# mitsuba-renderer/mitsuba2

Hardware: AMD Instinct MI355X
Metric: Msamples/sec (whole node), 1080p/512spp path integrator (higher is better)
Workload: dtype f32

## Files before the change

### mitsuba2_amd/csrc/device/film_kernels.h

```cpp
__global__ void k_film_resolve(const double *accum, float *out32, double *out64, size_t n, int accumulate) {
    size_t i = (size_t) blockIdx.x * blockDim.x + threadIdx.x;
    if (i >= n) return;
    if (out64) out64[i] = accumulate ? out64[i] + accum[i] : accum[i];
    else out32[i] = accumulate ? (float) ((double) out32[i] + accum[i]) : (float) accum[i];
}

#define MIW_FP_SIDE 8
#define MIW_FP_MAXN 8
struct PatchArgs { uint32_t patches_x, patches_y; int32_t reach; };

template <bool wide>
__global__ __launch_bounds__(64) void k_film_blocks(FilmRec F, BlockReplayArgs A, PatchArgs PA, float *tiles) {
    __shared__ float s_lut[MIW_FILTER_RESOLUTION + 1];
    __shared__ float s_w[64 * 2 * MIW_FP_MAXN];
    const uint32_t l = threadIdx.x;
    const uint32_t tile = blockIdx.x / (PA.patches_x * PA.patches_y), patch = blockIdx.x % (PA.patches_x * PA.patches_y);
    const uint32_t b = A.tile_list ? A.tile_list[tile] : tile;
    const BlockGeom g = block_geom(F, A.blocks_x, b);
    const int ptx0 = (int) (patch % PA.patches_x) * MIW_FP_SIDE, pty0 = (int) (patch / PA.patches_x) * MIW_FP_SIDE;
    if (ptx0 >= g.size_x || pty0 >= g.size_y) return;
    const int tx = ptx0 + (int) (l & 7u), ty = pty0 + (int) (l >> 3);
    if (l < 32) s_lut[l] = F.lut[l];
    __syncthreads();

// ... 563 lines not shown
#pragma unroll
            for (int p = P0; p <= P1; ++p) { wx[p].x = px[2 * p]; wx[p].y = px[2 * p + 1]; }
#pragma unroll
            for (int q = R0; q <= R1; ++q) {
                const float wy = py[q];
#pragma unroll
                for (int p = P0; p <= P1; ++p) {
                    const miw_f2 w = wy * wx[p];
                    film_pk_acc(acc[q][p][0], vx * w); film_pk_acc(acc[q][p][1], vy * w); film_pk_acc(acc[q][p][2], vz * w);
                    film_pk_acc(acc[q][p][3], af * w);
                    film_pk_acc(acc[q][p][4], w);
                }
#if MIW_FL_FENCE
                __builtin_amdgcn_sched_barrier(0);
#endif
            }
        }
    }
}
#ifndef MIW_FL_WAVES
#define MIW_FL_WAVES 3
#endif
template <int U, int NT, int WV = MIW_FL_WAVES>
__global__ __launch_bounds__(64) __attribute__((amdgpu_waves_per_eu(WV, 8))) void k_film_lanes(FilmRec F, BlockReplayArgs A, PatchArgs PA , uint32_t n_tiles, float *tiles,
                  uint32_t group0 ,
                  uint32_t prio ) {
    if (prio == 3u) __builtin_amdgcn_s_setprio(3); else if (prio == 2u) __builtin_amdgcn_s_setprio(2); else if (prio == 1u) __builtin_amdgcn_s_setprio(1);
    constexpr int BS = MIW_FL_BS, WS = MIW_FQ_WSTRIDE(MIW_FL_BS), LEAD = BS - 1, LCAP = 64;
    extern __shared__ float s_w[];
    __shared__ unsigned short s_list[LCAP];
    const uint32_t l = threadIdx.x;
    const uint32_t n_pos = PA.patches_x * PA.patches_y;
    const uint32_t tw = blockIdx.x / n_pos + group0, pos = blockIdx.x % n_pos;
    const int tx0 = (int) (pos % PA.patches_x) * BS, ty0 = (int) (pos / PA.patches_x) * BS;
    const uint32_t tile = tw * 64u + l;
    const bool live = tile < n_tiles;
    const BlockGeom g = block_geom(F, A.blocks_x, live ? (A.tile_list ? A.tile_list[tile] : tile) : 0u);
    const uint32_t rej = A.cls.count;
    const int reach = A.cls.reach;
    for (uint32_t i = l; i < (rej + 1u) * WS; i += 64u) {
        const uint32_t c = i / WS, a = i % WS;
        s_w[i] = (c < rej && a >= (uint32_t) LEAD && a <= (uint32_t) LEAD + 2u * (uint32_t) reach) ? A.cls.w[c * MIW_FC_STRIDE + a - LEAD] : 0.f;
    }
    const uint32_t bs2 = 1u << A.bs2_log2;
    uint32_t fill = 0;
    for (uint32_t q0 = 0; q0 < bs2; q0 += 64u) {
        const uint32_t q = q0 + l;
        uint32_t x, y;
        morton_decode2(q, x, y);
        const bool in = q < bs2 && (int) x >= tx0 - F.border - reach && (int) x <= tx0 + BS - 1 - F.border + reach &&
                        (int) y >= ty0 - F.border - reach && (int) y <= ty0 + BS - 1 - F.border + reach;
        const unsigned long long m = __ballot(in);
        if (in) {
            const uint32_t at = fill + (uint32_t) __popcll(m & ((1ull << l) - 1ull));
            if (at < (uint32_t) LCAP) s_list[at] = (unsigned short) q;
        }
        fill += (uint32_t) __popcll(m);
    }
    const uint32_t n_list = fill < (uint32_t) LCAP ? fill : (uint32_t) LCAP;
    __syncthreads();

    miw_f2 acc[BS][BS / 2][MIW_FILM_CHANNELS];
#pragma unroll
    for (int r = 0; r < BS; ++r)
#pragma unroll
        for (int p = 0; p < BS / 2; ++p)
#pragma unroll
            for (int k = 0; k < MIW_FILM_CHANNELS; ++k) acc[r][p][k] = (miw_f2) (0.f);
    const uint32_t w_base = (uint32_t) (uintptr_t) (miw_lds_cf *) s_w;
    const uint32_t off_rej = rej * (uint32_t) (WS * 4);
    const uint32_t lane0 = tile << A.bs2_log2;
    const uint32_t js = A.log_il ? 64u : 1u;
    struct Step { const U4 *run; uint32_t cnt; };
    auto pixel_at = [&](uint32_t k) { return (uint32_t) __builtin_amdgcn_readfirstlane((int) (k < n_list ? (uint32_t) s_list[k] : 0u)); };
    auto step_of = [&](uint32_t k, uint32_t q) {
        Step s; s.run = A.log_rec; s.cnt = 0u;
        uint32_t x, y;
        morton_decode2(q, x, y);
        if (k < n_list && live && (int) x < g.bw && (int) y < g.bh) { s.cnt = A.st[lane0 + q].w; s.run = A.log_rec + log_index(A.log_il, lane0 + q, A.spp, 0u); }
        return s;
    };
    uint4 nxt[U];
    auto fetch = [&](const U4 *run, uint32_t cnt) {
        const uint32_t last = cnt ? cnt - 1u : 0u;
#pragma unroll
        for (int i = 0; i < U; ++i) {
            nxt[i] = film_load_rec<NT>(run + ((uint32_t) i < last ? (uint32_t) i : last) * js);
            __builtin_amdgcn_sched_barrier(0);
        }
    };
    uint32_t q = pixel_at(0u);
    Step cur = step_of(0u, q);
    fetch(cur.run, cur.cnt);
    for (uint32_t k = 0; k < n_list; ++k) {
        const uint32_t step_max = (uint32_t) __builtin_amdgcn_readfirstlane((int) wave_max_u32(cur.cnt));
        const uint32_t qn = pixel_at(k + 1u);
        const Step nx = step_of(k + 1u, qn);
        uint32_t x, y;
        morton_decode2(q, x, y);
        const int ax = tx0 - ((int) x + F.border - reach), ay = ty0 - ((int) y + F.border - reach);
        const int c0 = ax < 0 ? -ax : 0, c1 = 2 * reach - ax < BS - 1 ? 2 * reach - ax : BS - 1;
        const int r0 = ay < 0 ? -ay : 0, r1 = 2 * reach - ay < BS - 1 ? 2 * reach - ay : BS - 1;
        const uint32_t bxa = w_base + 4u * (uint32_t) (LEAD + ax), bya = w_base + 4u * (uint32_t) (LEAD + ay);
        const int code = __builtin_amdgcn_readfirstlane(((r0 * 4 + r1) * 2 + (c0 >> 1)) * 2 + (c1 >> 1));
#define MIW_FL_CASE(R0, R1, P0, P1) case ((R0 * 4 + R1) * 2 + P0) * 2 + P1: \
            film_lanes_pixel<R0, R1, P0, P1, U, NT>(acc, nxt, cur.cnt, nx.run, nx.cnt, cur.run, step_max, bxa, bya, off_rej, js); break;
#define MIW_FL_ROWS(R0, R1) MIW_FL_CASE(R0, R1, 0, 0) MIW_FL_CASE(R0, R1, 0, 1) MIW_FL_CASE(R0, R1, 1, 1)
        switch (code) {
            MIW_FL_ROWS(0, 0) MIW_FL_ROWS(0, 1) MIW_FL_ROWS(0, 2) MIW_FL_ROWS(0, 3) MIW_FL_ROWS(1, 1) MIW_FL_ROWS(1, 2) MIW_FL_ROWS(1, 3)
            MIW_FL_ROWS(2, 2) MIW_FL_ROWS(2, 3) MIW_FL_ROWS(3, 3)
            default: break;
        }
#undef MIW_FL_ROWS
#undef MIW_FL_CASE
        if (step_max == 0u) fetch(nx.run, nx.cnt);
        cur = nx; q = qn;
    }
#pragma unroll
    for (int r = 0; r < BS; ++r)
#pragma unroll
        for (int c = 0; c < BS; ++c)
            if (live && tx0 + c < g.size_x && ty0 + r < g.size_y) {
                float *out = tiles + (size_t) tile * A.tile_stride + ((size_t) (ty0 + r) * g.size_x + (tx0 + c)) * MIW_FILM_CHANNELS;
#pragma unroll
                for (int k = 0; k < MIW_FILM_CHANNELS; ++k) out[k] = (c & 1) ? acc[r][c / 2][k].y : acc[r][c / 2][k].x;
            }
}

__global__ void k_film_merge(FilmRec F, BlockReplayArgs A, const float *tiles, float *out32, double *out64, int accumulate) {
    int fx = (int) (blockIdx.x * blockDim.x + threadIdx.x), fy = (int) blockIdx.y;
    if (fx >= F.crop_w || fy >= F.crop_h) return;
    float v[MIW_FILM_CHANNELS];
    size_t o = ((size_t) fy * F.crop_w + fx) * MIW_FILM_CHANNELS;
    if (accumulate) for (int k = 0; k < MIW_FILM_CHANNELS; ++k) v[k] = out64 ? (float) out64[o + k] : out32[o + k];
    film_merge_texel(F, A, tiles, fx, fy, v, accumulate != 0);
    for (int k = 0; k < MIW_FILM_CHANNELS; ++k) {
        if (out64) out64[o + k] = (double) v[k]; else out32[o + k] = v[k];
    }
}
```

### mitsuba2_amd/csrc/miwave.hip

```cpp
#include <hip/hip_runtime.h>
#include <stdio.h>
#include <stdlib.h>
#include <string.h>
#include <stdarg.h>
#include <string>
#include <vector>
#include <chrono>
#include <atomic>
#include <cmath>
#include <map>
#include <string>
#include <algorithm>

#include "../../include/miwave.h"
#if defined(MIW_SECTION_PROFILE)
__device__ unsigned long long g_sections[16];
#endif
#if defined(MIW_PHASE_STATS)
__device__ unsigned long long g_phase_stats[15];
#endif
#if defined(MIW_WALK_STATS)
__device__ unsigned long long g_walk_stats[8];
__device__ float g_walk_statsf[8];
#endif
// ... 4 lines not shown
#if defined(MIW_SECTION_PROFILE) && defined(__HIP_DEVICE_COMPILE__)
__device__ __forceinline__ unsigned long long *miw_sec_buf() { __shared__ unsigned long long b[4][16]; return &b[threadIdx.x >> 6][0]; }
#define MIW_SECTION(i) do { const unsigned long long now_ = __builtin_amdgcn_s_memtime(); unsigned long long *b_ = miw_sec_buf(); \
        if ((threadIdx.x & 63u) == (unsigned) __ffsll((long long) __ballot(1)) - 1u) { b_[i] += now_ - b_[15]; b_[15] = now_; } } while (0)
#endif
#include "miw/base.h"
#include "miw/rng.h"
#include "miw/warp.h"
#include "miw/special.h"
#include "miw/shape.h"
#include "miw/bsdf.h"
#include "miw/scene.h"
#include "miw/film.h"
#include "miw/bvh.h"
#include "miw/path.h"
#include "miw/direct.h"
#include "rect_build.h"
#include "miw/film_gather.h"
#include "texture_build.h"
#include "bvh_build.h"
#include "bvh4_build.h"
#include "envmap_build.h"
#include "film_classes.h"
#include "lbvh_device.h"
#include "sah_device.h"
#include "bvh4_device.h"
#include "bvh8_device.h"
#include "film_reduce.h"

using namespace miw;

static_assert(sizeof(BvhNode) == 64, "BvhNode must be one 64-byte line");
static_assert(sizeof(Tri) == 48, "Tri must be 48 bytes");
static_assert(sizeof(BsdfRec) == 128 && sizeof(mi_bsdf) == 128, "bsdf record layout");
static_assert(sizeof(TexRec) == sizeof(mi_texture), "texture record layout");

#define MIW_BLOCK 256
#ifndef MIW_POOL_NW
#define MIW_POOL_NW 12
#endif
#define MIW_CNT_SHARDS 1024
#define MIW_BRUTE_MAX_LEAF 2
#define MIW_BRUTE_MAX_TRIS 64
#define MIW_PLACE_PIECES 4

#include "device/trace.h"
// ... 49 lines not shown
    { "MIW_PHASED", "0: tree scenes take the lock-step kernel instead of the phase machine" },
    { "MIW_PHASED_WAVES", "3 | 4: wavefronts per SIMD the phase machine is launched for" },
    { "MIW_TRIO", "0: MATS_PLAIN kernels where the MATS_TRIO class would do" },
    { "MIW_SHADE_VOTE", "num:den of the phase machine's shade vote" },
    { "MIW_LOOP_EXIT", "node:triangle hand-over ratios of the phase machine's walk loops" },
    { "MIW_POOLED", "1: tree scenes take k_path_pooled (walk jobs pooled across the workgroup; experimental, slower: DESIGN.md)" },
    { "MIW_POOL_SHAPE", "12x1 | 8x2: wavefronts per workgroup x pixels per lane of k_path_pooled" },
    { "MIW_POOL_VOTE", "shade_min:walk_min:node_min:tri_min:claim_min of k_path_pooled" },
    { "MIW_TAIL_PRIO", "0: no least-progress-first wave priorities" },
    { "MIW_WG_PER_CU", "workgroups per CU of the packet kernels' persistent grid" },
    { "MIW_PLACE", "0: shards of about one pixel per lane skip the measuring launch + placed queues" },
    { "MIW_JOB_CHUNK", "smallest chunk of a full frame's pixel jobs, in samples (a power of two; default 64, the phase machine 32): the pixels' sample streams are cut into halving chunks drawn chunk-major from one queue; 0: a job = all the samples of a pixel" },
    { "MIW_JOB_CHUNK_FORCE", "1: chunk jobs whatever the frame's size (tests of the hand-over between lanes)" },
    { "MIW_PACKET_SHARD4", "0: a plain-diffuse packet job of at most four wavefronts of pixels per SIMD keeps the five-wavefront (96-register) kernel" },
    { "MIW_PLACE_MEASURE", "divisor: the measuring launch runs spp / divisor samples" },
    { "MIW_PLACE_SPREAD", "0 | 1: placed pieces = consecutive sorted lanes | one lane of every cost stratum" },
    { "MIW_STREAM", "0: plan 1 walks with one kernel per list slice instead of the persistent stream kernel" },
    { "MIW_FILM_LEGACY", "1: the 24-byte position log + k_film_blocks for every filter" },
    { "MIW_FILM_LANES", "0 | 1 | 2: k_film_lanes off / over the tile-interleaved log / over [lane][sample]" },
    { "MIW_FILM_QUADS", "0 | 24 | 28 | 42 | 44: k_film_quads group shape (0: off)" },
    { "MIW_FILM_COLUMNS", "0 | 42 | 44 | 82: k_film_columns group shape" },
    { "MIW_FILM_GROUP", "2 | 3 | 4: k_film_groups group shape" },
    { "MIW_FL_NT", "0: k_film_lanes reads the log with plain instead of streaming loads" },
    { "MIW_FILM_OVERLAP", "1: part of the film replay of a full Cornell-class frame is queued on three more streams beside the path kernel, sets of 64-tile groups each behind the flags their last pixels raise (default 0: measured +0 - 1 %); 2: without the waits (timing probe: the film is the previous frame's)" },
    { "MIW_FILM_OVERLAP_SET", "groups of 64 tiles per launch of that replay (default 4)" },
    { "MIW_FILM_OVERLAP_ROOM", "workgroups the path kernel's grid is short of filling the device while the replay runs beside it (default 32: one per CU on 32 CUs)" },
    { "MIW_FILM_OVERLAP_LEAN", "0: the launches of that replay are the 168-register kernel (default 1: the 128-register form)" },
    { "MIW_FILM_OVERLAP_BESIDE", "groups of 64 tiles replayed beside the path kernel; the rest in one launch after it (default: three quarters)" },
    { "MIW_FILM_OVERLAP_PRIO", "s_setprio of the replay wavefronts that run beside the path kernel, 0 .. 3 (default 0)" },
    { "MIW_FQ_U", "2 | 4 | 8: records per trip of k_film_quads" },
    { "MIW_RCCL", "0: mi_film_reduce never uses RCCL (device add)" },
    { "MIW_RCCL_FORCE", "1: mi_film_reduce takes the RCCL branch for one context too (tests)" }
};
struct Options {
    std::map<std::string, std::string> v;
    void from_env() { for (const KnobInfo &k : g_knobs) if (const char *e = getenv(k.name)) v[k.name] = e; }
    static bool known(const char *name) { for (const KnobInfo &k : g_knobs) if (!strcmp(k.name, name)) return true; return false; }
    const char *get(const char *name) const { auto it = v.find(name); return it == v.end() ? nullptr : it->second.c_str(); }
};

struct mi_ctx {
    int device = 0;
    Options opt;
    hipStream_t stream = nullptr;
    std::string error;
    std::atomic<int> cancel{0};
// ... 19 lines not shown
    DevBuf<float> d_env_data, d_env_levels; DevBuf<EnvmapRec> d_env; EnvmapRec env_host{}; size_t env_levels_total = 0;
    bool have_env = false;
    SceneView view{};
    TraceLds lds_cfg{}; size_t lds_bytes = 0;

    DevBuf<F4> q_tp, q_res, q_ray_o, q_ray_d, q_hit, q_sh_d, q_sh_c;
    DevBuf<U4> q_st; DevBuf<F2> q_pos; DevBuf<uint32_t> q_pixel, q_sh_vis;
    DevBuf<double> d_accum; DevBuf<unsigned char> d_out;
    DevBuf<F2> q_log_pos; DevBuf<F4> q_log_val;
    DevBuf<U4> q_log_rec;
    FilmClasses classes; FilmRec classes_of{}; bool classes_valid = false;
    DevBuf<float> d_fc_thr, d_fc_w;
    DevBuf<uint32_t> d_next_pixel; int cu_count = 256;
    DevBuf<uint32_t> d_lane_cost, d_cost_sorted, d_lane_iota, d_lane_sorted, d_piece_list, d_simd_ids;
    DevBuf<unsigned char> d_place_tmp;
    DevBuf<uint32_t> d_lists, d_list_counts;
    DevBuf<uint32_t> d_block_ids, d_tile_list; DevBuf<int32_t> d_block_tile; DevBuf<float> d_tiles;
    DevBuf<Counters> d_cnt;
    Counters *h_cnt = nullptr;
    std::vector<uint32_t> h_piece_list, h_simd_ids;
    hipStream_t stream2[3] = { nullptr, nullptr, nullptr }; hipEvent_t ev_fork = nullptr, ev_join[3] = { nullptr, nullptr, nullptr };
    DevBuf<uint32_t> d_group_done, d_group_expected; uint32_t *h_group_flag = nullptr; uint32_t group_flag_cap = 0;
    std::vector<uint32_t> h_group_expected; std::vector<int32_t> h_block_tile;
    int overlap_state = -1;
    bool replay_enqueued = false;
    uint32_t replay_launches = 0;

    std::vector<hipEvent_t> ev_pool;
    mi_counters counters{};
};

static mi_status fail(mi_ctx *c, mi_status code, const char *fmt, ...) {
    char buf[512];
    va_list ap; va_start(ap, fmt); vsnprintf(buf, sizeof buf, fmt, ap); va_end(ap);
    if (c) c->error = buf;
    return code;
}
#define HIP_TRY(c, expr) do { hipError_t e_ = (expr); if (e_ != hipSuccess) \
    return fail(c, MI_ERR_DEVICE, "%s failed: %s (%s:%d)", #expr, hipGetErrorString(e_), __FILE__, __LINE__); } while (0)

static thread_local std::string g_global_error;

extern "C" {

int32_t mi_spectrum_channels(void) { return MIW_SPEC_N; }

// ... 12 lines not shown
    int n = 0;
    if (hipGetDeviceCount(&n) != hipSuccess || n <= 0) { g_global_error = "no HIP device visible"; return MI_ERR_DEVICE; }
    if (device < 0 || device >= n) { g_global_error = "device index out of range"; return MI_ERR_INVALID; }
    if (hipSetDevice(device) != hipSuccess) { g_global_error = "hipSetDevice failed"; return MI_ERR_DEVICE; }
    mi_ctx *c = new mi_ctx();
    c->device = device;
    c->opt.from_env();
    { hipDeviceProp_t prop; if (hipGetDeviceProperties(&prop, device) == hipSuccess && prop.multiProcessorCount > 0) c->cu_count = prop.multiProcessorCount; }
    if (hipHostMalloc((void **) &c->h_cnt, sizeof(Counters) * MIW_CNT_SHARDS) != hipSuccess) { delete c; g_global_error = "hipHostMalloc failed"; return MI_ERR_DEVICE; }
    *out = c;
    g_live_contexts.fetch_add(1);
    return MI_OK;
}

void mi_destroy(mi_ctx *c) {
    if (!c) return;
    (void) hipSetDevice(c->device);
    (void) hipDeviceSynchronize();
    c->d_nodes.release(); c->d_tris.release(); c->d_tri_vn.release(); c->d_tri_uv.release(); c->d_bitmap_data.release(); c->d_bitmaps.release(); c->d_bsdf_tables.release(); c->d_shapes.release(); c->d_rects.release(); c->d_bsdfs.release();
    c->d_emitters.release(); c->d_leaf_boxes.release(); c->d_tri_bounds.release(); c->d_nodes4.release(); c->d_nodes8.release(); c->d_tris8.release(); c->d_tri_vn8.release(); c->d_env_data.release(); c->d_env_levels.release(); c->d_env.release(); c->d_emit_tri.release(); c->d_emit_vnorm.release(); c->d_emit_pmf.release(); c->d_emit_cdf.release();
    c->q_tp.release(); c->q_res.release(); c->q_ray_o.release(); c->q_ray_d.release(); c->q_hit.release();
    c->q_sh_d.release(); c->q_sh_c.release(); c->q_st.release(); c->q_pos.release(); c->q_pixel.release(); c->q_sh_vis.release();
    c->d_accum.release(); c->d_out.release(); c->d_next_pixel.release(); c->d_lane_cost.release(); c->d_cost_sorted.release(); c->d_lane_iota.release(); c->d_lane_sorted.release(); c->d_place_tmp.release(); c->d_piece_list.release(); c->d_simd_ids.release(); c->d_lists.release(); c->d_list_counts.release(); c->d_block_ids.release(); c->d_tile_list.release(); c->d_cnt.release();
    c->q_log_pos.release(); c->q_log_val.release(); c->q_log_rec.release(); c->d_fc_thr.release(); c->d_fc_w.release(); c->d_block_tile.release(); c->d_tiles.release();
    for (hipEvent_t e : c->ev_pool) (void) hipEventDestroy(e);
    c->d_group_done.release(); c->d_group_expected.release();
    if (c->h_group_flag) (void) hipHostFree(c->h_group_flag);
    if (c->ev_fork) (void) hipEventDestroy(c->ev_fork);
    for (int i = 0; i < 3; ++i) { if (c->ev_join[i]) (void) hipEventDestroy(c->ev_join[i]); if (c->stream2[i]) (void) hipStreamDestroy(c->stream2[i]); }
    if (c->h_cnt) (void) hipHostFree(c->h_cnt);
    delete c;
    if (g_live_contexts.fetch_sub(1) == 1) rccl_release_comms();
}

mi_status mi_set_stream(mi_ctx *c, void *s) { if (!c) return MI_ERR_INVALID; c->stream = (hipStream_t) s; return MI_OK; }

const char *mi_last_error(mi_ctx *c) { return c ? c->error.c_str() : g_global_error.c_str(); }

mi_status mi_set_option(mi_ctx *c, const char *name, const char *value) {
    if (!c || !name) return MI_ERR_INVALID;
    if (!Options::known(name)) return fail(c, MI_ERR_INVALID, "mi_set_option: unknown option %s", name);
    if (value) c->opt.v[name] = value; else c->opt.v.erase(name);
    return MI_OK;
}
const char *mi_get_option(mi_ctx *c, const char *name) { return c && name ? c->opt.get(name) : nullptr; }
int32_t mi_option_count(void) { return (int32_t) (sizeof(g_knobs) / sizeof(g_knobs[0])); }
const char *mi_option_name(int32_t i) { return i >= 0 && i < mi_option_count() ? g_knobs[i].name : nullptr; }
// ... 964 lines not shown
                }
                memset(st, 0, sizeof st); memset(stf, 0, sizeof stf);
                (void) hipMemcpyToSymbol(HIP_SYMBOL(g_walk_stats), st, sizeof st); (void) hipMemcpyToSymbol(HIP_SYMBOL(g_walk_statsf), stf, sizeof stf);
            }
        }
#endif
#if defined(MIW_SECTION_PROFILE)
        if (ropt.get("MIW_DEBUG")) {
            unsigned long long sec[16];
            if (hipMemcpyFromSymbol(sec, HIP_SYMBOL(g_sections), sizeof sec) == hipSuccess) {
                static const char *names[13] = { "fetch/begin", "leaf boxes", "E candidates", "S candidates", "path_step", "finish+begin",
                                                 "walks + votes", "shade: surface interaction", "shade: emitter hit + MIS", "shade: RR + emitter sampling + bsdf eval",
                                                 "shade: bsdf sample", "shade: finish + next sample", "shade: pixel fetch + walk start" };
                unsigned long long tot = 0;
                for (int i = 0; i < 13; ++i) tot += sec[i];
                for (int i = 0; i < 13; ++i) if (sec[i]) fprintf(stderr, "[miwave] section %-40s %6.2f %%\n", names[i], 100.0 * (double) sec[i] / (double) std::max<unsigned long long>(tot, 1));
                memset(sec, 0, sizeof sec);
                (void) hipMemcpyToSymbol(HIP_SYMBOL(g_sections), sec, sizeof sec);
            }
        }
#endif
}

struct FilmReplay { BlockReplayArgs A; uint32_t side = 0; uint32_t beside = 0;  };
static mi_status film_replay_setup(mi_ctx *c, const mi_render_cfg *cfg, hipStream_t s, const FilmPlan &FP, uint32_t n_tiles, uint32_t bs, uint32_t bs2_log2,
                                   uint32_t blocks_x, uint32_t blocks_y, FilmReplay &R) {
    const bool rec16 = FP.rec16;
    std::vector<int32_t> &block_tile = c->h_block_tile;
    block_tile.assign(cfg->block_count, -1);
    for (uint32_t t = 0; t < n_tiles; ++t) block_tile[cfg->tile_list ? cfg->tile_list[t] : t] = (int32_t) t;
    HIP_TRY(c, c->d_block_tile.resize(cfg->block_count));
    HIP_TRY(c, hipMemcpyAsync(c->d_block_tile.p, block_tile.data(), block_tile.size() * sizeof(int32_t), hipMemcpyHostToDevice, s));
    BlockReplayArgs &A = R.A;
    A.log_pos = c->q_log_pos.p; A.log_val = c->q_log_val.p; A.st = c->q_st.p; A.spp = cfg->spp;
    A.log_rec = rec16 ? c->q_log_rec.p : nullptr; A.log_il = rec16 ? FP.log_il : 0u;
    A.cls.thr = c->d_fc_thr.p; A.cls.w = c->d_fc_w.p; A.cls.count = rec16 ? c->classes.count : 0u; A.cls.reach = rec16 ? c->classes.reach : 0;
    A.block_ids = c->d_block_ids.p; A.block_tile = c->d_block_tile.p;
    A.tile_list = cfg->tile_list ? c->d_tile_list.p : nullptr;
    A.blocks_x = blocks_x; A.blocks_y = blocks_y; A.bs2_log2 = bs2_log2;
    R.side = bs + 2u * (uint32_t) cfg->filter_border;
    A.tile_stride = R.side * R.side * MIW_FILM_CHANNELS;
    HIP_TRY(c, c->d_tiles.resize((size_t) std::max<uint32_t>(n_tiles, 1) * A.tile_stride));
    return MI_OK;
}

__global__ void k_raise_flags(uint32_t *flag, uint32_t n) {
    const uint32_t i = blockIdx.x * blockDim.x + threadIdx.x;
    if (i < n) __hip_atomic_store(flag + i, 1u, __ATOMIC_RELEASE, __HIP_MEMORY_SCOPE_SYSTEM);
}
static mi_status overlap_prepare(mi_ctx *c, const mi_render_cfg *cfg, hipStream_t s, uint32_t n_tiles, uint32_t bs, uint32_t blocks_x, LaneQueues &Q, uint32_t bs2_log2) {
    const uint32_t n_groups = (n_tiles + 63u) / 64u;
    if (!c->ev_fork) {
        bool ok = hipEventCreateWithFlags(&c->ev_fork, hipEventDisableTiming) == hipSuccess;
        for (int i = 0; i < 3 && ok; ++i)
            ok = hipStreamCreateWithFlags(&c->stream2[i], hipStreamNonBlocking) == hipSuccess && hipEventCreateWithFlags(&c->ev_join[i], hipEventDisableTiming) == hipSuccess;
        if (!ok) { (void) hipGetLastError(); c->overlap_state = 0; return MI_OK; }
    }
    if (c->group_flag_cap < n_groups) {
        if (c->h_group_flag) (void) hipHostFree(c->h_group_flag);
        c->h_group_flag = nullptr; c->group_flag_cap = 0;
        const uint32_t cap = std::max<uint32_t>(1024u, n_groups);
        if (hipHostMalloc((void **) &c->h_group_flag, cap * sizeof(uint32_t), hipHostMallocCoherent | hipHostMallocMapped) != hipSuccess) { (void) hipGetLastError(); c->overlap_state = 0; return MI_OK; }
        c->group_flag_cap = cap;
    }
    std::vector<uint32_t> &expected = c->h_group_expected;
    expected.assign(n_groups, 0u);
    for (uint32_t t = 0; t < n_tiles; ++t) {
        const uint32_t b = cfg->tile_list ? cfg->tile_list[t] : t, bx = b % blocks_x, by = b / blocks_x;
        const int32_t bw = std::min<int32_t>((int32_t) bs, cfg->crop_w - (int32_t) (bx * bs)), bh = std::min<int32_t>((int32_t) bs, cfg->crop_h - (int32_t) (by * bs));
        expected[t >> 6] += (uint32_t) (std::max(bw, 0) * std::max(bh, 0));
    }
    HIP_TRY(c, c->d_group_done.resize(n_groups)); HIP_TRY(c, c->d_group_expected.resize(n_groups));
    memset(c->h_group_flag, 0, n_groups * sizeof(uint32_t));
    HIP_TRY(c, hipMemsetAsync(c->d_group_done.p, 0, n_groups * sizeof(uint32_t), s));
    HIP_TRY(c, hipMemcpyAsync(c->d_group_expected.p, expected.data(), n_groups * sizeof(uint32_t), hipMemcpyHostToDevice, s));
    Q.group_done = c->d_group_done.p; Q.group_expected = c->d_group_expected.p; Q.group_flag = c->h_group_flag; Q.group_shift = bs2_log2 + 6u;
    return MI_OK;
}
static mi_status overlap_enqueue(mi_ctx *c, const Options &ropt, const RenderParams &P, hipStream_t s, LaunchTimer &T, FilmReplay &R, uint32_t n_tiles, bool wait_flags) {
    const uint32_t n_all = (n_tiles + 63u) / 64u;
    uint32_t n_groups = n_all * 3u / 4u;
    if (const char *e = ropt.get("MIW_FILM_OVERLAP_BESIDE")) n_groups = (uint32_t) std::min<long>(std::max<long>(atol(e), 0), (long) n_all);
    int prio = 0;
    if (const char *e = ropt.get("MIW_FILM_OVERLAP_PRIO")) prio = std::min(3, std::max(0, atoi(e)));
    PatchArgs PC; PC.patches_x = PC.patches_y = (R.side + MIW_FL_BS - 1) / MIW_FL_BS; PC.reach = c->classes.reach;
    const uint32_t n_pos = PC.patches_x * PC.patches_y;
    const size_t lbytes = (size_t) (c->classes.count + 1u) * MIW_FQ_WSTRIDE(MIW_FL_BS) * sizeof(float);
    int fl_nt = 1;
    if (const char *e = ropt.get("MIW_FL_NT")) fl_nt = atoi(e);
    uint32_t set = 4u;
    if (const char *e = ropt.get("MIW_FILM_OVERLAP_SET")) set = (uint32_t) std::max(1, atoi(e));
    bool lean_ok = fl_nt != 0;
    if (const char *e = ropt.get("MIW_FILM_OVERLAP_LEAN")) lean_ok = lean_ok && atoi(e) != 0;
    for (int i = 0; i < 3; ++i) HIP_TRY(c, hipStreamWaitEvent(c->stream2[i], c->ev_fork, 0));
    uint32_t launches = 0;
    for (uint32_t g0 = 0; g0 < n_groups; g0 += set, ++launches) {
        hipStream_t b = c->stream2[launches % 3u];
        const uint32_t g1 = std::min(n_groups, g0 + set);
        if (wait_flags)
            for (uint32_t g = g0; g < g1; ++g) {
                const hipError_t e = hipStreamWaitValue32(b, c->h_group_flag + g, 1u, hipStreamWaitValueGte, 0xffffffffu);
                if (e != hipSuccess) {
                    (void) hipGetLastError();
                    c->overlap_state = 0;
                    if (g == 0) return MI_OK;
                    return fail(c, MI_ERR_DEVICE, "hipStreamWaitValue32 failed mid-frame: %s", hipGetErrorString(e));
                }
            }
        size_t e0 = 0, e1 = 0;
        if (T.on) { HIP_TRY(c, T.get_event(e0)); HIP_TRY(c, hipEventRecord(c->ev_pool[e0], b)); }
        const bool lean = lean_ok;
        if (lean) hipLaunchKernelGGL((k_film_lanes<2, 1, 4>), dim3((g1 - g0) * n_pos), dim3(64), lbytes, b, P.film, R.A, PC, (uint32_t) n_tiles, c->d_tiles.p, g0, (uint32_t) prio);
        else if (fl_nt) hipLaunchKernelGGL((k_film_lanes<4, 1>), dim3((g1 - g0) * n_pos), dim3(64), lbytes, b, P.film, R.A, PC, (uint32_t) n_tiles, c->d_tiles.p, g0, (uint32_t) prio);
        else hipLaunchKernelGGL((k_film_lanes<4, 0>), dim3((g1 - g0) * n_pos), dim3(64), lbytes, b, P.film, R.A, PC, (uint32_t) n_tiles, c->d_tiles.p, g0, (uint32_t) prio);
        if (T.on) { HIP_TRY(c, T.get_event(e1)); HIP_TRY(c, hipEventRecord(c->ev_pool[e1], b)); T.stamps.push_back({ 4, e0, e1 }); }
    }
    for (int i = 0; i < 3; ++i) HIP_TRY(c, hipEventRecord(c->ev_join[i], c->stream2[i]));
    c->replay_launches = launches;
    R.beside = n_groups;
    hipLaunchKernelGGL(k_raise_flags, dim3((n_all + 255u) / 256u), dim3(256), 0, s, c->h_group_flag, n_all);
    HIP_TRY(c, hipGetLastError());
    c->replay_enqueued = true;
    c->overlap_state = 1;
    return MI_OK;
}

static mi_status assemble_film(mi_ctx *c, const mi_render_cfg *cfg, const Options &ropt, const RenderParams &P, hipStream_t s, LaunchTimer &T, const FilmPlan &FP,
                               uint32_t n_tiles, uint32_t bs, uint32_t bs2_log2, uint32_t blocks_x, uint32_t blocks_y, size_t film_n, void *film, mi_status result,
                               const FilmReplay *queued ) {
    const int film_mode = FP.film_mode; const bool rec16 = FP.rec16; const int film_lanes = FP.film_lanes; const uint32_t log_il = FP.log_il;
    (void) result;
#define MIW_TIMED(cls_, launch) do {                                                   \
        size_t e0_ = 0, e1_ = 0;                                                       \
        if (T.on) { HIP_TRY(c, T.get_event(e0_)); HIP_TRY(c, hipEventRecord(c->ev_pool[e0_], s)); } \
        launch;                                                                        \
        if (T.on) { HIP_TRY(c, T.get_event(e1_)); HIP_TRY(c, hipEventRecord(c->ev_pool[e1_], s)); \
                    T.stamps.push_back({ cls_, e0_, e1_ }); }                          \
    } while (0)
    {
        const size_t elem = cfg->film_f64 ? sizeof(double) : sizeof(float);
        void *dst = film;
        const bool staged = !cfg->film_on_device;
        if (staged) {
            HIP_TRY(c, c->d_out.resize(film_n * elem)); dst = c->d_out.p;
            if (cfg->accumulate) HIP_TRY(c, hipMemcpyAsync(c->d_out.p, film, film_n * elem, hipMemcpyHostToDevice, s));
        }
        float *dst32 = cfg->film_f64 ? nullptr : (float *) dst;
        double *dst64 = cfg->film_f64 ? (double *) dst : nullptr;
        if (film_mode == 1) {
            FilmReplay R;
            if (queued) R = *queued;
            else { const mi_status rs = film_replay_setup(c, cfg, s, FP, n_tiles, bs, bs2_log2, blocks_x, blocks_y, R); if (rs != MI_OK) return rs; }
            BlockReplayArgs &A = R.A;
            const uint32_t side = R.side;
            if (n_tiles) {
                PatchArgs PA;
                PA.patches_x = PA.patches_y = (side + MIW_FP_SIDE - 1) / MIW_FP_SIDE;
                PA.reach = (int32_t) floorf(cfg->filter_radius + .5f);
                const dim3 fgrid(n_tiles * PA.patches_x * PA.patches_y);
                const bool wide = cfg->filter_radius > 0.5f + MIW_RAY_EPSILON;
                if (rec16) {
                    int group = 3;
                    if (const char *e = ropt.get("MIW_FILM_GROUP")) group = atoi(e);
                    const size_t wbytes = (size_t) (c->classes.count + 1u) * MIW_FG_WSTRIDE * sizeof(float);
#define MIW_FG_LAUNCH(GW, GH) MIW_TIMED(4, hipLaunchKernelGGL((k_film_groups<GW, GH>), fgrid, dim3(64), wbytes, s, P.film, A, PA, c->d_tiles.p))
#define MIW_FC_LAUNCH(GW, GH) do { PatchArgs PC = PA; PC.patches_x = (side + (GW) - 1) / (GW); PC.patches_y = (side + (GH) - 1) / (GH); \
                                   const uint32_t per_wave = 64u / (GW), wpt = (PC.patches_x * PC.patches_y + per_wave - 1u) / per_wave; \
                                   MIW_TIMED(4, hipLaunchKernelGGL((k_film_columns<GW, GH>), dim3(n_tiles * wpt), dim3(64), wbytes, s, P.film, A, PC, c->d_tiles.p)); } while (0)
                    int columns = 42;
                    if (const char *e = ropt.get("MIW_FILM_COLUMNS")) columns = atoi(e);
                    int quads = ropt.get("MIW_FILM_COLUMNS") == nullptr && ropt.get("MIW_FILM_GROUP") == nullptr ? 42 : 0;
                    if (const char *e = ropt.get("MIW_FILM_QUADS")) quads = atoi(e) == 1 ? 42 : atoi(e);
                    if ((quads != 24 && quads != 42 && quads != 28 && quads != 44) || c->classes.reach > 2) quads = 0;
                    const uint32_t qw = (uint32_t) quads / 10u, qh = (uint32_t) quads % 10u;
                    if (quads && ((side + qw - 1) / qw) * ((side + qh - 1) / qh) < 64u / qw) quads = 0;
                    const bool lanes = film_lanes != 0;
                    c->counters.film_kernel = lanes ? 4u : quads ? 3u : (columns == 42 || columns == 44 || columns == 82) ? 2u : 1u;
                    if (lanes) {
                        PatchArgs PC = PA; PC.patches_x = PC.patches_y = (side + MIW_FL_BS - 1) / MIW_FL_BS;
                        const size_t lbytes = (size_t) (c->classes.count + 1u) * MIW_FQ_WSTRIDE(MIW_FL_BS) * sizeof(float);
                        int fl_nt = 1;
                        if (const char *e = ropt.get("MIW_FL_NT")) fl_nt = atoi(e);
                        const uint32_t first = queued ? queued->beside : 0u, groups_all = ((uint32_t) n_tiles + 63u) / 64u;
                        const uint32_t waves_rest = (groups_all - first) * PC.patches_x * PC.patches_y;
                        if (waves_rest == 0u) { }
                        else if (fl_nt) MIW_TIMED(4, hipLaunchKernelGGL((k_film_lanes<4, 1>), dim3(waves_rest), dim3(64), lbytes, s, P.film, A, PC, (uint32_t) n_tiles, c->d_tiles.p, first, 0u));
                        else MIW_TIMED(4, hipLaunchKernelGGL((k_film_lanes<4, 0>), dim3(waves_rest), dim3(64), lbytes, s, P.film, A, PC, (uint32_t) n_tiles, c->d_tiles.p, first, 0u));
                        if (queued) { for (int i = 0; i < 3; ++i) HIP_TRY(c, hipStreamWaitEvent(s, c->ev_join[i], 0)); }
                    } else if (quads) {
                        PatchArgs PC = PA; PC.patches_x = (side + qw - 1) / qw; PC.patches_y = (side + qh - 1) / qh;
                        const uint32_t per_wave = 64u / qw, waves = (uint32_t) (((size_t) n_tiles * PC.patches_x * PC.patches_y + per_wave - 1u) / per_wave);
                        const size_t qbytes = (size_t) (c->classes.count + 1u) * (size_t) (5u + 2u * qh) * sizeof(float);
#define MIW_FQ_LAUNCH(GW, GH, U) MIW_TIMED(4, hipLaunchKernelGGL((k_film_quads<GW, GH, U>), dim3(waves), dim3(64), qbytes, s, P.film, A, PC, (uint32_t) n_tiles, c->d_tiles.p))
                        int fq_u = 4;
                        if (const char *e = ropt.get("MIW_FQ_U")) fq_u = atoi(e);
                        if (quads == 24) { if (fq_u == 8) MIW_FQ_LAUNCH(2, 4, 8); else if (fq_u == 2) MIW_FQ_LAUNCH(2, 4, 2); else MIW_FQ_LAUNCH(2, 4, 4); }
                        else if (quads == 42) { if (fq_u == 8) MIW_FQ_LAUNCH(4, 2, 8); else MIW_FQ_LAUNCH(4, 2, 4); }
                        else if (quads == 28) MIW_FQ_LAUNCH(2, 8, 4); else MIW_FQ_LAUNCH(4, 4, 4);
#undef MIW_FQ_LAUNCH
                    } else if (columns == 42) MIW_FC_LAUNCH(4, 2); else if (columns == 44) MIW_FC_LAUNCH(4, 4); else if (columns == 82) MIW_FC_LAUNCH(8, 2);
                    else if (group == 4) MIW_FG_LAUNCH(4, 4); else if (group == 2) MIW_FG_LAUNCH(2, 2); else MIW_FG_LAUNCH(4, 2);
#undef MIW_FC_LAUNCH
#undef MIW_FG_LAUNCH
                } else if (wide)
                    MIW_TIMED(4, hipLaunchKernelGGL(k_film_blocks<true>, fgrid, dim3(64), 0, s, P.film, A, PA, c->d_tiles.p));
                else
                    MIW_TIMED(4, hipLaunchKernelGGL(k_film_blocks<false>, fgrid, dim3(64), 0, s, P.film, A, PA, c->d_tiles.p));
            }
            MIW_TIMED(5, hipLaunchKernelGGL(k_film_merge, dim3(((uint32_t) cfg->crop_w + 255u) / 256u, (uint32_t) cfg->crop_h), dim3(256), 0, s,
                                            P.film, A, c->d_tiles.p, dst32, dst64, cfg->accumulate));
// ... 246 lines not shown
            TA.side = 16u + 2u * std::max<uint32_t>((uint32_t) cfg->filter_border, (uint32_t) floorf(cfg->filter_radius + .5f));
            TA.geom16 = (uint32_t) ((c->lds_bytes + 15) / 16);
            tile_bytes = (size_t) TA.geom16 * 16 - c->lds_bytes + (size_t) TA.side * TA.side * MIW_FILM_CHANNELS * sizeof(double);
            if (c->lds_bytes + tile_bytes > 64 * 1024) {
                HIP_TRY(c, hipFuncSetAttribute((const void *) k_path_resident<false, 1>, hipFuncAttributeMaxDynamicSharedMemorySize, (int) (c->lds_bytes + tile_bytes)));
                HIP_TRY(c, hipFuncSetAttribute((const void *) k_path_resident<false, 0>, hipFuncAttributeMaxDynamicSharedMemorySize, (int) (c->lds_bytes + tile_bytes)));
                HIP_TRY(c, hipFuncSetAttribute((const void *) k_path_resident<false, 1, MATS_ALL, false, INTEG_DIRECT>, hipFuncAttributeMaxDynamicSharedMemorySize, (int) (c->lds_bytes + tile_bytes)));
                HIP_TRY(c, hipFuncSetAttribute((const void *) k_path_resident<false, 0, MATS_ALL, true, INTEG_DIRECT>, hipFuncAttributeMaxDynamicSharedMemorySize, (int) (c->lds_bytes + tile_bytes)));
            }
        }
        const uint32_t sync_every = 8;
        uint32_t launches = 0;
        bool place_stats_due = false;
        int overlap_mode = 0;
        if (const char *e = ropt.get("MIW_FILM_OVERLAP")) overlap_mode = atoi(e);
        const bool overlap = overlap_mode != 0 && c->overlap_state != 0 && film_mode == 1 && FP.rec16 && FP.film_lanes != 0 && FP.log_il != 0 && !place && !phased  && tiny && c->diffuse_only && !MIW_SPECTRAL && !direct  &&
                             per_launch >= cfg->spp && cfg->timeout_s <= 0.f && n_tiles > 0;
        for (uint32_t done = 0; done < cfg->spp; ) {
            uint32_t end = cfg->spp - done < per_launch ? cfg->spp : done + per_launch;
            if (film_mode == 1) {
                HIP_TRY(c, hipMemsetAsync(c->d_next_pixel.p, 0, c->d_next_pixel.n * sizeof(uint32_t), s));
                rcfg.queues = 1u; Q.lane_cost = nullptr; Q.lane_sorted = nullptr; Q.piece_list = nullptr; Q.simd_ids = nullptr;
                if (overlap && done == 0) {
                    mi_status os = film_replay_setup(c, cfg, s, FP, n_tiles, bs, bs2_log2, blocks_x, blocks_y, replay);
                    if (os == MI_OK) os = overlap_prepare(c, cfg, s, n_tiles, bs, blocks_x, Q, bs2_log2);
                    if (os != MI_OK) return os;
                    if (Q.group_done) HIP_TRY(c, hipEventRecord(c->ev_fork, s));
                }
                Q.job_chunk = Q.job_pow = Q.job_total = 0u; Q.job_min = 0x80000000u;
                if ((tiny || (phased && MIW_PHASED_JOBS != 0)) && !pooled_fits && !place && !overlap && done == 0 && per_launch >= cfg->spp && cfg->timeout_s <= 0.f) {
                    uint32_t jmin = tiny ? 64u : 32u;
                    if (const char *e = ropt.get("MIW_JOB_CHUNK")) { const uint32_t v = (uint32_t) std::max(0, atoi(e)); jmin = (v & (v - 1u)) ? 0u : v; }
                    bool enough = (uint64_t) n_lanes * 5u >= (uint64_t) 6u * 64u * res_waves * n_simd;
                    if (const char *e = ropt.get("MIW_JOB_CHUNK_FORCE")) enough = enough || atoi(e) != 0;
                    uint32_t pow2 = 1u;
                    while (pow2 * 2u < cfg->spp) pow2 *= 2u;
                    uint64_t chunks = 1u;
                    for (uint32_t r = pow2; jmin && r >= jmin && r < cfg->spp; r >>= 1) ++chunks;
                    if (jmin && enough && chunks >= 2u && (uint64_t) n_lanes * chunks < (1ull << 31)) {
                        Q.job_chunk = jmin; Q.job_min = jmin; Q.job_pow = pow2; Q.job_total = (uint32_t) ((uint64_t) n_lanes * chunks);
                        K.job_chunk = jmin; K.job_chunks = (uint32_t) chunks;
                    }
                }
                if (place && done == 0) { end = measure_end; Q.lane_cost = c->d_lane_cost.p; Q.simd_ids = c->d_simd_ids.p; }
                else if (place) {
                    HIP_TRY(c, rocprim::radix_sort_pairs_desc(c->d_place_tmp.p, place_tmp_bytes, c->d_lane_cost.p, c->d_cost_sorted.p, c->d_lane_iota.p, c->d_lane_sorted.p, (size_t) n_lanes, 0u, 32u, s));
                    bool spread = phased && ((phased8 ? (size_t) c->nodes8_count * sizeof(Bvh8Node) : (size_t) c->nodes4_count * sizeof(Bvh4Node)) + (size_t) c->view.tri_count * sizeof(Tri)) > ((size_t) 32 << 20);
// ... 304 lines not shown
```

Measured before the change: 4467.

## Pack film-lane block positions into equal-length chains per wavefront

The film replay kernel now processes a chain of up to four block positions per wavefront instead of one. A host-side bin packer groups positions so each chain has roughly equal pixel work, flushing accumulators between positions. This balances work across wavefronts and reduces the number of short-lived workgroups for border positions. An optional U=8 variant with two waves per SIMD is also added, but only behind an option. The cost is extra LDS for four lists, per-position bookkeeping, and serialised flushes inside a wave.

```diff
diff --git a/mitsuba2_amd/csrc/device/film_kernels.h b/mitsuba2_amd/csrc/device/film_kernels.h
--- a/mitsuba2_amd/csrc/device/film_kernels.h
+++ b/mitsuba2_amd/csrc/device/film_kernels.h
@@ -609,17 +609,20 @@
 #define MIW_FL_WAVES 3
 #endif
 template <int U, int NT, int WV = MIW_FL_WAVES>
-__global__ __launch_bounds__(64) __attribute__((amdgpu_waves_per_eu(WV, 8))) void k_film_lanes(FilmRec F, BlockReplayArgs A, PatchArgs PA , uint32_t n_tiles, float *tiles,
+__global__ __launch_bounds__(64) __attribute__((amdgpu_waves_per_eu(WV, 8))) void k_film_lanes(FilmRec F, BlockReplayArgs A, PatchArgs PA ,
+                  const uint2 *chains , uint32_t n_chains ,
+                  uint32_t n_tiles, float *tiles,
                   uint32_t group0 ,
                   uint32_t prio ) {
     if (prio == 3u) __builtin_amdgcn_s_setprio(3); else if (prio == 2u) __builtin_amdgcn_s_setprio(2); else if (prio == 1u) __builtin_amdgcn_s_setprio(1);
     constexpr int BS = MIW_FL_BS, WS = MIW_FQ_WSTRIDE(MIW_FL_BS), LEAD = BS - 1, LCAP = 64;
     extern __shared__ float s_w[];
-    __shared__ unsigned short s_list[LCAP];
+    __shared__ unsigned short s_list[MIW_FL_CHAIN_POS][LCAP];
     const uint32_t l = threadIdx.x;
-    const uint32_t n_pos = PA.patches_x * PA.patches_y;
-    const uint32_t tw = blockIdx.x / n_pos + group0, pos = blockIdx.x % n_pos;
-    const int tx0 = (int) (pos % PA.patches_x) * BS, ty0 = (int) (pos / PA.patches_x) * BS;
+    const uint32_t tw = blockIdx.x / n_chains + group0;
+    const uint2 cw = chains[blockIdx.x % n_chains];
+    const uint32_t cpos0 = cw.x & 0xffffu, cpos1 = cw.x >> 16, cpos2 = cw.y & 0xffffu, cpos3 = cw.y >> 16;
+    auto pos_of = [&](uint32_t p) { return p == 0u ? cpos0 : p == 1u ? cpos1 : p == 2u ? cpos2 : cpos3; };
     const uint32_t tile = tw * 64u + l;
     const bool live = tile < n_tiles;
     const BlockGeom g = block_geom(F, A.blocks_x, live ? (A.tile_list ? A.tile_list[tile] : tile) : 0u);
@@ -630,21 +633,28 @@
         s_w[i] = (c < rej && a >= (uint32_t) LEAD && a <= (uint32_t) LEAD + 2u * (uint32_t) reach) ? A.cls.w[c * MIW_FC_STRIDE + a - LEAD] : 0.f;
     }
     const uint32_t bs2 = 1u << A.bs2_log2;
-    uint32_t fill = 0;
+    uint32_t fill[MIW_FL_CHAIN_POS] = { 0u, 0u, 0u, 0u };
     for (uint32_t q0 = 0; q0 < bs2; q0 += 64u) {
         const uint32_t q = q0 + l;
         uint32_t x, y;
         morton_decode2(q, x, y);
-        const bool in = q < bs2 && (int) x >= tx0 - F.border - reach && (int) x <= tx0 + BS - 1 - F.border + reach &&
-                        (int) y >= ty0 - F.border - reach && (int) y <= ty0 + BS - 1 - F.border + reach;
-        const unsigned long long m = __ballot(in);
-        if (in) {
-            const uint32_t at = fill + (uint32_t) __popcll(m & ((1ull << l) - 1ull));
-            if (at < (uint32_t) LCAP) s_list[at] = (unsigned short) q;
-        }
-        fill += (uint32_t) __popcll(m);
-    }
-    const uint32_t n_list = fill < (uint32_t) LCAP ? fill : (uint32_t) LCAP;
+#pragma unroll
+        for (int p = 0; p < MIW_FL_CHAIN_POS; ++p) {
+            const uint32_t pos = pos_of((uint32_t) p);
+            const int bx0 = (int) (pos % PA.patches_x) * BS, by0 = (int) (pos / PA.patches_x) * BS;
+            const bool in = pos != MIW_FL_CHAIN_NONE && q < bs2 && (int) x >= bx0 - F.border - reach && (int) x <= bx0 + BS - 1 - F.border + reach &&
+                            (int) y >= by0 - F.border - reach && (int) y <= by0 + BS - 1 - F.border + reach;
+            const unsigned long long m = __ballot(in);
+            if (in) {
+                const uint32_t at = fill[p] + (uint32_t) __popcll(m & ((1ull << l) - 1ull));
+                if (at < (uint32_t) LCAP) s_list[p][at] = (unsigned short) q;
+            }
+            fill[p] += (uint32_t) __popcll(m);
+        }
+    }
+    const uint32_t s1 = min(fill[0], (uint32_t) LCAP), s2 = s1 + min(fill[1], (uint32_t) LCAP), s3 = s2 + min(fill[2], (uint32_t) LCAP);
+    const uint32_t n_list = min(s3 + min(fill[3], (uint32_t) LCAP), (uint32_t) LCAP);
+    auto part_of = [&](uint32_t k) { return k < s1 ? 0u : k < s2 ? 1u : k < s3 ? 2u : 3u; };
     __syncthreads();
 
     miw_f2 acc[BS][BS / 2][MIW_FILM_CHANNELS];
@@ -659,7 +669,29 @@
     const uint32_t lane0 = tile << A.bs2_log2;
     const uint32_t js = A.log_il ? 64u : 1u;
     struct Step { const U4 *run; uint32_t cnt; };
-    auto pixel_at = [&](uint32_t k) { return (uint32_t) __builtin_amdgcn_readfirstlane((int) (k < n_list ? (uint32_t) s_list[k] : 0u)); };
+    auto pixel_at = [&](uint32_t k) {
+        const uint32_t p = part_of(k), k0 = p == 0u ? 0u : p == 1u ? s1 : p == 2u ? s2 : s3;
+        return (uint32_t) __builtin_amdgcn_readfirstlane((int) (k < n_list ? (uint32_t) s_list[p][k - k0] : 0u));
+    };
+    auto flush = [&](uint32_t p) {
+        const uint32_t pos = pos_of(p);
+        const int bx0 = (int) (pos % PA.patches_x) * BS, by0 = (int) (pos / PA.patches_x) * BS;
+#pragma unroll
+        for (int r = 0; r < BS; ++r)
+#pragma unroll
+            for (int c = 0; c < BS; ++c)
+                if (live && bx0 + c < g.size_x && by0 + r < g.size_y) {
+                    float *out = tiles + (size_t) tile * A.tile_stride + ((size_t) (by0 + r) * g.size_x + (bx0 + c)) * MIW_FILM_CHANNELS;
+#pragma unroll
+                    for (int k = 0; k < MIW_FILM_CHANNELS; ++k) out[k] = (c & 1) ? acc[r][c / 2][k].y : acc[r][c / 2][k].x;
+                }
+#pragma unroll
+        for (int r = 0; r < BS; ++r)
+#pragma unroll
+            for (int c = 0; c < BS / 2; ++c)
+#pragma unroll
+                for (int k = 0; k < MIW_FILM_CHANNELS; ++k) acc[r][c][k] = (miw_f2) (0.f);
+    };
     auto step_of = [&](uint32_t k, uint32_t q) {
         Step s; s.run = A.log_rec; s.cnt = 0u;
         uint32_t x, y;
@@ -679,7 +711,12 @@
     uint32_t q = pixel_at(0u);
     Step cur = step_of(0u, q);
     fetch(cur.run, cur.cnt);
+    uint32_t p_cur = part_of(0u);
     for (uint32_t k = 0; k < n_list; ++k) {
+        const uint32_t pk = part_of(k);
+        if (pk != p_cur) { flush(p_cur); p_cur = pk; }
+        const uint32_t pos = pos_of(pk);
+        const int tx0 = (int) (pos % PA.patches_x) * BS, ty0 = (int) (pos / PA.patches_x) * BS;
         const uint32_t step_max = (uint32_t) __builtin_amdgcn_readfirstlane((int) wave_max_u32(cur.cnt));
         const uint32_t qn = pixel_at(k + 1u);
         const Step nx = step_of(k + 1u, qn);
@@ -703,15 +740,10 @@
         if (step_max == 0u) fetch(nx.run, nx.cnt);
         cur = nx; q = qn;
     }
-#pragma unroll
-    for (int r = 0; r < BS; ++r)
-#pragma unroll
-        for (int c = 0; c < BS; ++c)
-            if (live && tx0 + c < g.size_x && ty0 + r < g.size_y) {
-                float *out = tiles + (size_t) tile * A.tile_stride + ((size_t) (ty0 + r) * g.size_x + (tx0 + c)) * MIW_FILM_CHANNELS;
-#pragma unroll
-                for (int k = 0; k < MIW_FILM_CHANNELS; ++k) out[k] = (c & 1) ? acc[r][c / 2][k].y : acc[r][c / 2][k].x;
-            }
+    if (n_list) flush(p_cur);
+#pragma unroll
+    for (int p = 0; p < MIW_FL_CHAIN_POS; ++p)
+        if (pos_of((uint32_t) p) != MIW_FL_CHAIN_NONE && fill[p] == 0u) flush((uint32_t) p);
 }
 
 __global__ void k_film_merge(FilmRec F, BlockReplayArgs A, const float *tiles, float *out32, double *out64, int accumulate) {
diff --git a/mitsuba2_amd/csrc/film_chains.h b/mitsuba2_amd/csrc/film_chains.h
--- /dev/null
+++ b/mitsuba2_amd/csrc/film_chains.h
@@ -0,0 +1,44 @@
+#pragma once
+#include <stdint.h>
+#include <algorithm>
+#include <vector>
+
+#define MIW_FL_CHAIN_POS 4
+#define MIW_FL_CHAIN_NONE 0xffffu
+
+inline uint32_t film_chain_span(int t0, int bs, int border, int reach) {
+    const int lo = std::max(t0 - border - reach, 0), hi = std::min(t0 + 3 - border + reach, bs - 1);
+    return hi >= lo ? (uint32_t) (hi - lo + 1) : 0u;
+}
+
+inline uint32_t film_chain_pixels(uint32_t pos, uint32_t patches, int bs, int border, int reach) {
+    return film_chain_span((int) (pos % patches) * 4, bs, border, reach) * film_chain_span((int) (pos / patches) * 4, bs, border, reach);
+}
+
+inline std::vector<uint64_t> film_lane_chains(uint32_t bs, int border, int reach, bool equal) {
+    const uint32_t side = bs + 2u * (uint32_t) border, patches = (side + 3u) / 4u, n_pos = patches * patches;
+    std::vector<uint64_t> out;
+    auto pack = [](const std::vector<uint32_t> &ids) {
+        uint64_t w = 0;
+        for (int i = 0; i < MIW_FL_CHAIN_POS; ++i) w |= (uint64_t) (i < (int) ids.size() ? ids[i] : MIW_FL_CHAIN_NONE) << (16 * i);
+        return w;
+    };
+    if (!equal) {
+        for (uint32_t p = 0; p < n_pos; ++p) out.push_back(pack({ p }));
+        return out;
+    }
+    std::vector<uint32_t> cnt(n_pos), order(n_pos);
+    uint32_t cap = 1;
+    for (uint32_t p = 0; p < n_pos; ++p) { cnt[p] = film_chain_pixels(p, patches, (int) bs, border, reach); order[p] = p; cap = std::max(cap, cnt[p]); }
+    std::stable_sort(order.begin(), order.end(), [&](uint32_t a, uint32_t b) { return cnt[a] > cnt[b]; });
+    std::vector<std::vector<uint32_t>> bins;
+    std::vector<uint32_t> load;
+    for (uint32_t p : order) {
+        size_t b = 0;
+        while (b < bins.size() && (bins[b].size() >= (size_t) MIW_FL_CHAIN_POS || load[b] + cnt[p] > cap)) ++b;
+        if (b == bins.size()) { bins.emplace_back(); load.push_back(0u); }
+        bins[b].push_back(p); load[b] += cnt[p];
+    }
+    for (const auto &ids : bins) out.push_back(pack(ids));
+    return out;
+}
diff --git a/mitsuba2_amd/csrc/miwave.hip b/mitsuba2_amd/csrc/miwave.hip
--- a/mitsuba2_amd/csrc/miwave.hip
+++ b/mitsuba2_amd/csrc/miwave.hip
@@ -50,6 +50,7 @@
 #include "bvh4_build.h"
 #include "envmap_build.h"
 #include "film_classes.h"
+#include "film_chains.h"
 #include "lbvh_device.h"
 #include "sah_device.h"
 #include "bvh4_device.h"
@@ -145,6 +146,8 @@
     { "MIW_FILM_COLUMNS", "0 | 42 | 44 | 82: k_film_columns group shape" },
     { "MIW_FILM_GROUP", "2 | 3 | 4: k_film_groups group shape" },
     { "MIW_FL_NT", "0: k_film_lanes reads the log with plain instead of streaming loads" },
+    { "MIW_FL_CHAINS", "0: k_film_lanes replays one block position per wavefront instead of chains of equal length (film_chains.h)" },
+    { "MIW_FL_U", "8: k_film_lanes with eight records in flight per lane, compiled for two wavefronts per SIMD (default 4, three wavefronts)" },
     { "MIW_FILM_OVERLAP", "1: part of the film replay of a full Cornell-class frame is queued on three more streams beside the path kernel, sets of 64-tile groups each behind the flags their last pixels raise (default 0: measured +0 - 1 %); 2: without the waits (timing probe: the film is the previous frame's)" },
     { "MIW_FILM_OVERLAP_SET", "groups of 64 tiles per launch of that replay (default 4)" },
     { "MIW_FILM_OVERLAP_ROOM", "workgroups the path kernel's grid is short of filling the device while the replay runs beside it (default 32: one per CU on 32 CUs)" },
@@ -210,6 +213,7 @@
     hipStream_t stream2[3] = { nullptr, nullptr, nullptr }; hipEvent_t ev_fork = nullptr, ev_join[3] = { nullptr, nullptr, nullptr };
     DevBuf<uint32_t> d_group_done, d_group_expected; uint32_t *h_group_flag = nullptr; uint32_t group_flag_cap = 0;
     std::vector<uint32_t> h_group_expected; std::vector<int32_t> h_block_tile;
+    std::vector<uint64_t> h_fl_chains; DevBuf<uint2> d_fl_chains; uint64_t fl_chains_key = ~0ull;
     int overlap_state = -1;
     bool replay_enqueued = false;
     uint32_t replay_launches = 0;
@@ -268,7 +272,7 @@
     c->q_tp.release(); c->q_res.release(); c->q_ray_o.release(); c->q_ray_d.release(); c->q_hit.release();
     c->q_sh_d.release(); c->q_sh_c.release(); c->q_st.release(); c->q_pos.release(); c->q_pixel.release(); c->q_sh_vis.release();
     c->d_accum.release(); c->d_out.release(); c->d_next_pixel.release(); c->d_lane_cost.release(); c->d_cost_sorted.release(); c->d_lane_iota.release(); c->d_lane_sorted.release(); c->d_place_tmp.release(); c->d_piece_list.release(); c->d_simd_ids.release(); c->d_lists.release(); c->d_list_counts.release(); c->d_block_ids.release(); c->d_tile_list.release(); c->d_cnt.release();
-    c->q_log_pos.release(); c->q_log_val.release(); c->q_log_rec.release(); c->d_fc_thr.release(); c->d_fc_w.release(); c->d_block_tile.release(); c->d_tiles.release();
+    c->q_log_pos.release(); c->q_log_val.release(); c->q_log_rec.release(); c->d_fc_thr.release(); c->d_fc_w.release(); c->d_block_tile.release(); c->d_tiles.release(); c->d_fl_chains.release();
     for (hipEvent_t e : c->ev_pool) (void) hipEventDestroy(e);
     c->d_group_done.release(); c->d_group_expected.release();
     if (c->h_group_flag) (void) hipHostFree(c->h_group_flag);
@@ -1279,8 +1283,9 @@
 #endif
 }
 
-struct FilmReplay { BlockReplayArgs A; uint32_t side = 0; uint32_t beside = 0;  };
-static mi_status film_replay_setup(mi_ctx *c, const mi_render_cfg *cfg, hipStream_t s, const FilmPlan &FP, uint32_t n_tiles, uint32_t bs, uint32_t bs2_log2,
+struct FilmReplay { BlockReplayArgs A; uint32_t side = 0; uint32_t beside = 0;
+                    const uint2 *chains = nullptr; uint32_t n_chains = 0;  };
+static mi_status film_replay_setup(mi_ctx *c, const mi_render_cfg *cfg, const Options &ropt, hipStream_t s, const FilmPlan &FP, uint32_t n_tiles, uint32_t bs, uint32_t bs2_log2,
                                    uint32_t blocks_x, uint32_t blocks_y, FilmReplay &R) {
     const bool rec16 = FP.rec16;
     std::vector<int32_t> &block_tile = c->h_block_tile;
@@ -1298,6 +1303,18 @@
     R.side = bs + 2u * (uint32_t) cfg->filter_border;
     A.tile_stride = R.side * R.side * MIW_FILM_CHANNELS;
     HIP_TRY(c, c->d_tiles.resize((size_t) std::max<uint32_t>(n_tiles, 1) * A.tile_stride));
+    if (rec16 && FP.film_lanes) {
+        bool equal = true;
+        if (const char *e = ropt.get("MIW_FL_CHAINS")) equal = atoi(e) != 0;
+        const uint64_t key = (uint64_t) bs | (uint64_t) (uint32_t) cfg->filter_border << 16 | (uint64_t) (uint32_t) c->classes.reach << 32 | (uint64_t) equal << 48;
+        if (key != c->fl_chains_key || !c->d_fl_chains.p) {
+            c->h_fl_chains = film_lane_chains(bs, cfg->filter_border, c->classes.reach, equal);
+            HIP_TRY(c, c->d_fl_chains.resize(c->h_fl_chains.size()));
+            HIP_TRY(c, hipMemcpyAsync(c->d_fl_chains.p, c->h_fl_chains.data(), c->h_fl_chains.size() * sizeof(uint64_t), hipMemcpyHostToDevice, s));
+            c->fl_chains_key = key;
+        }
+        R.chains = c->d_fl_chains.p; R.n_chains = (uint32_t) c->h_fl_chains.size();
+    }
     return MI_OK;
 }
 
@@ -1341,7 +1358,7 @@
     int prio = 0;
     if (const char *e = ropt.get("MIW_FILM_OVERLAP_PRIO")) prio = std::min(3, std::max(0, atoi(e)));
     PatchArgs PC; PC.patches_x = PC.patches_y = (R.side + MIW_FL_BS - 1) / MIW_FL_BS; PC.reach = c->classes.reach;
-    const uint32_t n_pos = PC.patches_x * PC.patches_y;
+    const uint32_t n_pos = R.n_chains;
     const size_t lbytes = (size_t) (c->classes.count + 1u) * MIW_FQ_WSTRIDE(MIW_FL_BS) * sizeof(float);
     int fl_nt = 1;
     if (const char *e = ropt.get("MIW_FL_NT")) fl_nt = atoi(e);
@@ -1367,9 +1384,9 @@
         size_t e0 = 0, e1 = 0;
         if (T.on) { HIP_TRY(c, T.get_event(e0)); HIP_TRY(c, hipEventRecord(c->ev_pool[e0], b)); }
         const bool lean = lean_ok;
-        if (lean) hipLaunchKernelGGL((k_film_lanes<2, 1, 4>), dim3((g1 - g0) * n_pos), dim3(64), lbytes, b, P.film, R.A, PC, (uint32_t) n_tiles, c->d_tiles.p, g0, (uint32_t) prio);
-        else if (fl_nt) hipLaunchKernelGGL((k_film_lanes<4, 1>), dim3((g1 - g0) * n_pos), dim3(64), lbytes, b, P.film, R.A, PC, (uint32_t) n_tiles, c->d_tiles.p, g0, (uint32_t) prio);
-        else hipLaunchKernelGGL((k_film_lanes<4, 0>), dim3((g1 - g0) * n_pos), dim3(64), lbytes, b, P.film, R.A, PC, (uint32_t) n_tiles, c->d_tiles.p, g0, (uint32_t) prio);
+        if (lean) hipLaunchKernelGGL((k_film_lanes<2, 1, 4>), dim3((g1 - g0) * n_pos), dim3(64), lbytes, b, P.film, R.A, PC, R.chains, R.n_chains, (uint32_t) n_tiles, c->d_tiles.p, g0, (uint32_t) prio);
+        else if (fl_nt) hipLaunchKernelGGL((k_film_lanes<4, 1>), dim3((g1 - g0) * n_pos), dim3(64), lbytes, b, P.film, R.A, PC, R.chains, R.n_chains, (uint32_t) n_tiles, c->d_tiles.p, g0, (uint32_t) prio);
+        else hipLaunchKernelGGL((k_film_lanes<4, 0>), dim3((g1 - g0) * n_pos), dim3(64), lbytes, b, P.film, R.A, PC, R.chains, R.n_chains, (uint32_t) n_tiles, c->d_tiles.p, g0, (uint32_t) prio);
         if (T.on) { HIP_TRY(c, T.get_event(e1)); HIP_TRY(c, hipEventRecord(c->ev_pool[e1], b)); T.stamps.push_back({ 4, e0, e1 }); }
     }
     for (int i = 0; i < 3; ++i) HIP_TRY(c, hipEventRecord(c->ev_join[i], c->stream2[i]));
@@ -1407,7 +1424,7 @@
         if (film_mode == 1) {
             FilmReplay R;
             if (queued) R = *queued;
-            else { const mi_status rs = film_replay_setup(c, cfg, s, FP, n_tiles, bs, bs2_log2, blocks_x, blocks_y, R); if (rs != MI_OK) return rs; }
+            else { const mi_status rs = film_replay_setup(c, cfg, ropt, s, FP, n_tiles, bs, bs2_log2, blocks_x, blocks_y, R); if (rs != MI_OK) return rs; }
             BlockReplayArgs &A = R.A;
             const uint32_t side = R.side;
             if (n_tiles) {
@@ -1439,10 +1456,13 @@
                         int fl_nt = 1;
                         if (const char *e = ropt.get("MIW_FL_NT")) fl_nt = atoi(e);
                         const uint32_t first = queued ? queued->beside : 0u, groups_all = ((uint32_t) n_tiles + 63u) / 64u;
-                        const uint32_t waves_rest = (groups_all - first) * PC.patches_x * PC.patches_y;
+                        const uint32_t waves_rest = (groups_all - first) * R.n_chains;
+                        int fl_u = 4;
+                        if (const char *e = ropt.get("MIW_FL_U")) fl_u = atoi(e);
                         if (waves_rest == 0u) { }
-                        else if (fl_nt) MIW_TIMED(4, hipLaunchKernelGGL((k_film_lanes<4, 1>), dim3(waves_rest), dim3(64), lbytes, s, P.film, A, PC, (uint32_t) n_tiles, c->d_tiles.p, first, 0u));
-                        else MIW_TIMED(4, hipLaunchKernelGGL((k_film_lanes<4, 0>), dim3(waves_rest), dim3(64), lbytes, s, P.film, A, PC, (uint32_t) n_tiles, c->d_tiles.p, first, 0u));
+                        else if (fl_nt && fl_u == 8) MIW_TIMED(4, hipLaunchKernelGGL((k_film_lanes<8, 1, 2>), dim3(waves_rest), dim3(64), lbytes, s, P.film, A, PC, R.chains, R.n_chains, (uint32_t) n_tiles, c->d_tiles.p, first, 0u));
+                        else if (fl_nt) MIW_TIMED(4, hipLaunchKernelGGL((k_film_lanes<4, 1>), dim3(waves_rest), dim3(64), lbytes, s, P.film, A, PC, R.chains, R.n_chains, (uint32_t) n_tiles, c->d_tiles.p, first, 0u));
+                        else MIW_TIMED(4, hipLaunchKernelGGL((k_film_lanes<4, 0>), dim3(waves_rest), dim3(64), lbytes, s, P.film, A, PC, R.chains, R.n_chains, (uint32_t) n_tiles, c->d_tiles.p, first, 0u));
                         if (queued) { for (int i = 0; i < 3; ++i) HIP_TRY(c, hipStreamWaitEvent(s, c->ev_join[i], 0)); }
                     } else if (quads) {
                         PatchArgs PC = PA; PC.patches_x = (side + qw - 1) / qw; PC.patches_y = (side + qh - 1) / qh;
@@ -1735,7 +1755,7 @@
                 HIP_TRY(c, hipMemsetAsync(c->d_next_pixel.p, 0, c->d_next_pixel.n * sizeof(uint32_t), s));
                 rcfg.queues = 1u; Q.lane_cost = nullptr; Q.lane_sorted = nullptr; Q.piece_list = nullptr; Q.simd_ids = nullptr;
                 if (overlap && done == 0) {
-                    mi_status os = film_replay_setup(c, cfg, s, FP, n_tiles, bs, bs2_log2, blocks_x, blocks_y, replay);
+                    mi_status os = film_replay_setup(c, cfg, ropt, s, FP, n_tiles, bs, bs2_log2, blocks_x, blocks_y, replay);
                     if (os == MI_OK) os = overlap_prepare(c, cfg, s, n_tiles, bs, blocks_x, Q, bs2_log2);
                     if (os != MI_OK) return os;
                     if (Q.group_done) HIP_TRY(c, hipEventRecord(c->ev_fork, s));
```

New measurement: 4472 (median of 6 runs). Within noise of the previous version (+0.1%).
